# flanglet/kanzi-go

Measured on AMD Instinct MI355X. Metric: encode+decode MB/s (round trip of the whole stream, uncompressed 10^6 B per second), higher is better.
Workload: dtype u8

## Files before the change

kanzi-go_amd/csrc/ans1.hip:

```cpp
#include "bits.h"

#define KNZ_ANS1_CHUNK (4u << 20)
#define KNZ_ANS1_LR 11
#define KNZ_ANS1_SCALE 2048
#define KNZ_ANS1_LDS_MAX_CHUNKS 1280u
#define KNZ_ANS1_CTXHDR_BYTES 448
#define KNZ_ANS1_U0_CAP (256 * KNZ_ANS1_CTXHDR_BYTES + 64)
#define KNZ_ANS1_U1_OFF KNZ_ANS1_U0_CAP
#define KNZ_ANS1_PAY_OFF (KNZ_ANS1_U0_CAP + 64)
#define KNZ_ANS1_PAY_CAP (((KNZ_ANS1_CHUNK / 8) * 11) + 64)
#define KNZ_ANS1_SLOT (KNZ_ANS1_PAY_OFF + KNZ_ANS1_PAY_CAP + 64)
#define KNZ_ANS1_CUM_STRIDE 257
#define KNZ_ANS1_PAYRING 8192
#define KNZ_ANS1_RING 2048

struct Ans1Args {
    const uint64_t* blk_off;
    const uint32_t* blk_len;
    uint32_t chunks_per_block;
    uint32_t nslots;
    uint8_t* scratch;
    uint32_t* unit_bits;
    uint32_t* unit_src;
    uint32_t* freqs;
// ... 304 lines not shown
        flush(m0, m1, m2);
    }
    const uint32_t s1 = wave_shfl(st, 1), s2 = wave_shfl(st, 2), s3 = wave_shfl(st, 3);
    if (bad && lane == 0) a.blk_status[b] = KNZ_ERR_PROCESS_BLOCK;
    if (live && lane == 0) {
        const uint32_t end4 = n & ~3u;
        const uint32_t tail = n & 3;
        for (uint32_t i = 0; i < tail; i++) payEnd[i] = src[end4 + i];
        const uint32_t nbytes = 2 * flushed + tail;
        uint32_t w[8];
        for (int i = 0; i < 8; i++) w[i] = 0;
        KnzBitWriter bw;
        bw.init(w);
        knz_put_varint(bw, nbytes);
        bw.put(st, 32); bw.put(s1, 32); bw.put(s2, 32); bw.put(s3, 32);
        uint32_t* u1 = (uint32_t*)(slot + KNZ_ANS1_U1_OFF);
        for (int i = 0; i < 8; i++) u1[i] = knz_bswap32(w[i]);
        uint32_t* ubits = a.unit_bits + (size_t)slotId * KNZ_UNITS_PER_CHUNK;
        uint32_t* usrc = a.unit_src + (size_t)slotId * KNZ_UNITS_PER_CHUNK;
        ubits[1] = bw.pos;
        ubits[2] = 8 * nbytes;
        usrc[2] = (uint32_t)(KNZ_ANS1_PAY_OFF + KNZ_ANS1_PAY_CAP - 2 * flushed);
    }
}

#ifndef KNZ_HIP_EMU
#define KNZ_A1E_SDWA " dst_sel:DWORD dst_unused:UNUSED_PAD src0_sel:DWORD src1_sel:WORD_1\n\t"
#define KNZ_A1E_STEP(J, A, B) \
    "v_cmp_ge_u32_e32 vcc, %[" A "], %[y" J "]\n\t" \
    "v_cndmask_b32_sdwa %[t], %[" A "], %[" A "], vcc" KNZ_A1E_SDWA \
    "v_mul_hi_u32 %[q], %[t], %[x" J "]\n\t" \
    "v_lshrrev_b32_e32 %[q], %[w" J "], %[q]\n\t" \
    "v_mul_u32_u24_sdwa %[q], %[q], %[w" J "]" KNZ_A1E_SDWA \
    "v_add3_u32 %[" B "], %[t], %[z" J "], %[q]\n\t"
__device__ __forceinline__ void knz_a1e_run4(uint32_t& st, const uint4& e0, const uint4& e1, const uint4& e2, const uint4& e3, uint32_t* slot) {
    uint32_t q, t, s1, s2, s3, s4;
    asm volatile(KNZ_A1E_STEP("0", "s0", "s1") KNZ_A1E_STEP("1", "s1", "s2") KNZ_A1E_STEP("2", "s2", "s3") KNZ_A1E_STEP("3", "s3", "s4")
                 : [s1] "=&v"(s1), [s2] "=&v"(s2), [s3] "=&v"(s3), [s4] "=&v"(s4), [q] "=&v"(q), [t] "=&v"(t)
                 : [s0] "v"(st), [x0] "v"(e0.x), [y0] "v"(e0.y), [z0] "v"(e0.z), [w0] "v"(e0.w), [x1] "v"(e1.x), [y1] "v"(e1.y), [z1] "v"(e1.z), [w1] "v"(e1.w),
                   [x2] "v"(e2.x), [y2] "v"(e2.y), [z2] "v"(e2.z), [w2] "v"(e2.w), [x3] "v"(e3.x), [y3] "v"(e3.y), [z3] "v"(e3.z), [w3] "v"(e3.w)
                 : "vcc");
    uint4 sv; sv.x = st; sv.y = s1; sv.z = s2; sv.w = s3;
    *(uint4*)slot = sv;
    st = s4;
}
template <int R>
__device__ __forceinline__ void knz_a1e_run_group(uint32_t& st, const uint4* e, uint32_t* mine) {
    knz_a1e_run4(st, e[0], e[1], e[2], e[3], mine + R * 64);
    knz_a1e_run4(st, e[4], e[5], e[6], e[7], mine + R * 64 + 4);
    knz_a1e_run4(st, e[8], e[9], e[10], e[11], mine + R * 64 + 8);
    knz_a1e_run4(st, e[12], e[13], e[14], e[15], mine + R * 64 + 12);
}

__global__ __launch_bounds__(64) void knz_ans1_encode_asm_kernel(Ans1Args a, const uint4* ent) {
    __shared__ __attribute__((aligned(16))) uint32_t s_w[3 * KNZ_ANS1_GROUP * 4];
    const int lane = threadIdx.x;
    const uint32_t slotId = blockIdx.x;
    uint32_t b, n; const uint8_t* src; bool bad;
    const uint32_t steps = knz_ans1_steps(a, slotId, b, n, src, bad);
    const bool live = n != 0;
    uint8_t* slot = a.scratch + (size_t)slotId * KNZ_ANS1_SLOT;
    uint8_t* payEnd = slot + KNZ_ANS1_PAY_OFF + KNZ_ANS1_PAY_CAP;
    const uint4* __restrict__ base = ent + (size_t)slotId * KNZ_ANS1_ENT_STRIDE;
    const uint4* __restrict__ my = base + (size_t)(lane & 3);
    uint32_t* mine = s_w + 16 * (lane & 3);
    uint32_t st = 1u << 15;
    uint32_t flushed = 0;
    uint4 buf0[KNZ_ANS1_GROUP], buf1[KNZ_ANS1_GROUP], buf2[KNZ_ANS1_GROUP];
    uint32_t xm0 = 0xFFFFFFFFu, xm1 = 0xFFFFFFFFu, xm2;
    auto load_group = [&](uint32_t t0, uint4* e, uint32_t& xm) {
#pragma unroll
        for (int j = 0; j < KNZ_ANS1_GROUP; j++) e[j] = my[(size_t)(t0 + j) * 4];
        xm = base[(size_t)t0 * 4 + (uint32_t)lane].y;
    };
    auto flush = [&](uint32_t x0, uint32_t x1, uint32_t x2) {
        wave_sync_lds();
        const uint64_t below = ((uint64_t)1 << lane) - 1;
        const uint32_t fi = 16u * (uint32_t)(lane & 3) + (uint32_t)(lane >> 2);
        const uint32_t v0 = s_w[fi], v1 = s_w[64 + fi], v2 = s_w[128 + fi];
        const uint64_t m0 = wave_ballot(v0 >= x0), m1 = wave_ballot(v1 >= x1), m2 = wave_ballot(v2 >= x2);
        const uint32_t c0 = (uint32_t)__popcll(m0), c1 = (uint32_t)__popcll(m1), c2 = (uint32_t)__popcll(m2);
#pragma unroll
        for (int r = 0; r < 3; r++) {
            const uint64_t m = r == 0 ? m0 : (r == 1 ? m1 : m2);
            const uint32_t before = r == 0 ? 0u : (r == 1 ? c0 : c0 + c1);
            if ((m >> lane) & 1) {
                const uint32_t pos = flushed + before + (uint32_t)__popcll(m & below);
                const uint32_t wv = r == 0 ? v0 : (r == 1 ? v1 : v2);
                uint8_t* p = payEnd - 2 * ((size_t)pos + 1);
                p[0] = (uint8_t)(wv >> 8);
                p[1] = (uint8_t)wv;
            }
        }
        flushed += c0 + c1 + c2;
        wave_sync_lds();
    };
#pragma unroll
    for (int j = 0; j < KNZ_ANS1_GROUP; j++) { buf0[j].x = 0; buf0[j].y = 0xFFFFFFFFu; buf0[j].z = 0; buf0[j].w = 0; buf1[j] = buf0[j]; }
    for (uint32_t t0 = 0; t0 < steps + 2 * KNZ_ANS1_GROUP && steps; t0 += 3 * KNZ_ANS1_GROUP) {
        load_group(t0, buf2, xm2); knz_a1e_run_group<0>(st, buf0, mine);
        const uint32_t f0 = xm0;
        load_group(t0 + KNZ_ANS1_GROUP, buf0, xm0); knz_a1e_run_group<1>(st, buf1, mine);
        const uint32_t f1 = xm1;
        load_group(t0 + 2 * KNZ_ANS1_GROUP, buf1, xm1); knz_a1e_run_group<2>(st, buf2, mine);
        flush(f0, f1, xm2);
    }
    const uint32_t s1 = wave_shfl(st, 1), s2 = wave_shfl(st, 2), s3 = wave_shfl(st, 3);
    if (bad && lane == 0) a.blk_status[b] = KNZ_ERR_PROCESS_BLOCK;
    if (live && lane == 0) {
        const uint32_t end4 = n & ~3u;
        const uint32_t tail = n & 3;
        for (uint32_t i = 0; i < tail; i++) payEnd[i] = src[end4 + i];
        const uint32_t nbytes = 2 * flushed + tail;
        uint32_t w[8];
        for (int i = 0; i < 8; i++) w[i] = 0;
        KnzBitWriter bw;
        bw.init(w);
        knz_put_varint(bw, nbytes);
        bw.put(st, 32); bw.put(s1, 32); bw.put(s2, 32); bw.put(s3, 32);
        uint32_t* u1 = (uint32_t*)(slot + KNZ_ANS1_U1_OFF);
        for (int i = 0; i < 8; i++) u1[i] = knz_bswap32(w[i]);
        uint32_t* ubits = a.unit_bits + (size_t)slotId * KNZ_UNITS_PER_CHUNK;
        uint32_t* usrc = a.unit_src + (size_t)slotId * KNZ_UNITS_PER_CHUNK;
        ubits[1] = bw.pos;
        ubits[2] = 8 * nbytes;
        usrc[2] = (uint32_t)(KNZ_ANS1_PAY_OFF + KNZ_ANS1_PAY_CAP - 2 * flushed);
    }
}
#endif

struct Ans1DecArgs {
    const uint8_t* stream; uint64_t nbytes;
    const uint32_t* blk_pre_len;
    const uint8_t* blk_mode;
    const uint64_t* chunk_bit;
    const uint64_t* blk_out_off;
    uint32_t chunks_per_block;
    uint32_t nslots;
    uint32_t* dtab;
    uint32_t* info;
    uint64_t* paybit;
    int32_t* blk_status;
    uint32_t plain_loop;
    uint64_t* progress;
};

template <typename R>
__device__ static bool knz_ans1_parse_ctx(R& r, uint16_t* f, uint32_t llr, uint32_t scale, int& countOut) {
    uint8_t alpha[256];
    int count = 0;
    if (r.read(1) == 0) {
        if (r.read(1) == 1) count = 0;
        else { count = 256; if (f) for (int i = 0; i < 256; i++) alpha[i] = (uint8_t)i; }
    } else {
        const uint32_t lastMask = r.read(5);
        if (f) {
            for (uint32_t mm = 0; mm <= lastMask; mm++) {
                const uint32_t mask = r.read(8);
                for (int j = 0; j < 8; j++) if ((mask >> j) & 1) alpha[count++] = (uint8_t)(8 * mm + j);
            }
        } else {
            for (uint32_t bitsLeft = 8 * (lastMask + 1); bitsLeft > 0;) {
                const uint32_t take = bitsLeft > 32 ? 32 : bitsLeft;
                count += __popc(r.read(take));
                bitsLeft -= take;
            }
        }
    }
    countOut = count;
    if (count == 0) return true;
    const int chk = count < 64 ? 6 : 8;
    uint32_t sum = 0;
    for (int i = 1; i < count; i += chk) {
        const uint32_t logMax = r.read(llr);
        if ((1u << logMax) > scale) return false;
        const int endj = min(i + chk, count);
        if (!f) { r.skip_bits((uint32_t)(endj - i) * logMax); continue; }
        for (int j = i; j < endj; j++) {
            uint32_t fr = 1;
            if (logMax > 0) { fr = 1 + r.read(logMax); if (fr >= scale) return false; }
            f[alpha[j]] = (uint16_t)fr;
            sum += fr;
// ... 598 lines not shown
```

kanzi-go_amd/csrc/huffman_dec.hip:

```cpp
#include "bits.h"

struct KnzStreamReader {
    const uint32_t* words;
    uint64_t nwords;
    uint64_t next;
    uint64_t win;
    uint32_t navail;
    uint32_t pre;
    __device__ __forceinline__ uint32_t ld_raw(uint64_t i) const { return i < nwords ? words[i] : 0u; }
    __device__ __forceinline__ uint32_t ld(uint64_t i) const { return knz_bswap32(ld_raw(i)); }
    __device__ __forceinline__ void init(const uint8_t* base, uint64_t nbytes, uint64_t bitpos) {
        words = (const uint32_t*)base;
        nwords = (nbytes + 3) >> 2;
        uint64_t q = bitpos >> 5;
        uint32_t off = (uint32_t)(bitpos & 31);
        win = ((uint64_t)ld(q) << 32) | ld(q + 1);
        win <<= off;
        navail = 64 - off;
        next = q + 2;
        pre = ld_raw(next);
    }
    __device__ __forceinline__ void refill() {
        if (navail <= 32) { win |= (uint64_t)knz_bswap32(pre) << (32 - navail); navail += 32; next++; pre = ld_raw(next); }
    }
// ... 15 lines not shown
    uint64_t win;
    uint32_t navail;
    __device__ __forceinline__ void stage(uint64_t b) {
        const uint64_t l = (uint64_t)lane_id();
        base = b;
        w0 = (b + l < nwords) ? words[b + l] : 0u;
        w1 = (b + 64 + l < nwords) ? words[b + 64 + l] : 0u;
    }
    __device__ __forceinline__ uint32_t ld(uint64_t i) {
        if (i < base || i >= base + 128) stage(i);
        const uint32_t k = (uint32_t)(i - base);
        const uint32_t v = k < 64 ? wave_readlane(w0, k) : wave_readlane(w1, k - 64);
        return knz_bswap32(v);
    }
    __device__ __forceinline__ void init(const uint8_t* b, uint64_t nbytes, uint64_t bitpos) {
        words = (const uint32_t*)b;
        nwords = (nbytes + 3) >> 2;
        stage(bitpos >> 5);
        seek(bitpos);
    }
    __device__ __forceinline__ void seek(uint64_t bitpos) {
        const uint64_t q = bitpos >> 5;
        const uint32_t off = (uint32_t)(bitpos & 31);
        win = ((uint64_t)ld(q) << 32) | ld(q + 1);
        win <<= off;
        navail = 64 - off;
        next = q + 2;
    }
    __device__ __forceinline__ void refill() {
        if (navail <= 32) { win |= (uint64_t)ld(next++) << (32 - navail); navail += 32; }
    }
    __device__ __forceinline__ uint32_t peek(uint32_t n) { refill(); return (uint32_t)(win >> (64 - n)); }
    __device__ __forceinline__ void skip(uint32_t n) { refill(); win <<= n; navail -= n; }
    __device__ __forceinline__ void skip_bits(uint32_t n) { if (n <= 32) skip(n); else seek(tell() + n); }
    __device__ __forceinline__ uint32_t read(uint32_t n) { uint32_t v = peek(n); win <<= n; navail -= n; return v; }
    __device__ __forceinline__ uint64_t tell() const { return (next << 5) - navail; }
};

template <typename R>
__device__ __forceinline__ uint32_t knz_read_varint(R& r) {
    uint32_t res = 0, shift = 0;
    for (int i = 0; i < 4; i++) {
        uint32_t v = r.read(8);
        res |= (v & 0x7F) << shift;
        if (v < 128) return res;
        shift += 7;
    }
    uint32_t v = r.read(8);
    return res | ((v & 0x0F) << 28);
}

template <typename R>
__device__ static bool knz_ans1_parse_header(R& r, uint16_t* freq16, uint32_t& lrOut, int& totalAlpha, uint64_t* ctxpos, bool store);

struct WalkStreamArgs {
    const uint8_t* stream; uint64_t nbytes;
    uint64_t first_bit;
    uint64_t seg_bits;
    uint32_t max_blocks;
    uint64_t* blk_bit;
    uint64_t* blk_bits;
    uint32_t* result;
};

__global__ void knz_dec_walk_stream_kernel(WalkStreamArgs a) {
    if (threadIdx.x != 0 || blockIdx.x != 0) return;
    KnzStreamReader r;
    r.init(a.stream, a.nbytes, a.first_bit);
    const uint64_t limit = a.nbytes << 3;
    uint32_t n = 0, err = 0;
    for (;;) {
        if (a.seg_bits && r.tell() >= a.first_bit + a.seg_bits) break;
        if (r.tell() + 8 > limit) { err = KNZ_ERR_PROCESS_BLOCK; break; }
        uint32_t lr = r.read(5) + 3;
        uint64_t read = 0;
        if (lr > 32) { read = (uint64_t)r.read(lr - 32) << 32; read |= r.read(32); }
        else read = r.read(lr);
        if (read == 0) break;
        if (read > ((uint64_t)1 << 34)) { err = KNZ_ERR_BLOCK_SIZE; break; }
        uint64_t pos = r.tell();
        if (pos + read > limit) { err = KNZ_ERR_PROCESS_BLOCK; break; }
        if (n >= a.max_blocks) { err = KNZ_ERR_BLOCK_SIZE; break; }
        a.blk_bit[n] = pos;
        a.blk_bits[n] = read;
        n++;
        r.seek(pos + read);
    }
    a.result[0] = n;
    a.result[1] = err;
}

struct WalkRangeArgs {
    const uint8_t* stream; uint64_t nbytes;
    uint64_t first_bit;
    uint64_t first_id, from, to;
    uint32_t max_blocks;
    uint32_t cap;
    uint32_t frames;
    uint32_t stride;
    uint32_t hinted;
    uint64_t* blk_bit; uint64_t* blk_bits;
    uint64_t* result;
};

__global__ void knz_dec_walk_range_kernel(WalkRangeArgs a) {
    if (threadIdx.x != 0 || blockIdx.x != 0) return;
    KnzStreamReader r;
    r.init(a.stream, a.nbytes, a.first_bit);
    const uint64_t limit = a.nbytes << 3;
    uint64_t id = a.first_id, n = 0, end = 0;
    uint32_t seen = 0, err = 0;
    while (id < a.to) {
        const uint64_t at = r.tell();
        if (at + 8 > limit) { err = KNZ_ERR_PROCESS_BLOCK; break; }
        const uint32_t lr = r.read(5) + 3;
        uint64_t read = 0;
        if (lr > 32) { read = (uint64_t)r.read(lr - 32) << 32; read |= r.read(32); }
        else read = r.read(lr);
        const uint64_t pos = r.tell();
        if (read == 0) { end = pos; if (a.hinted && seen == 0) err = KNZ_ERR_PROCESS_BLOCK; break; }
        if (read > ((uint64_t)1 << 34)) { err = KNZ_ERR_BLOCK_SIZE; break; }
        if (pos + read > limit) { err = KNZ_ERR_PROCESS_BLOCK; break; }
        if (seen >= a.max_blocks) { err = KNZ_ERR_BLOCK_SIZE; break; }
        seen++;
        if (id >= a.from) {
            if (n < a.cap) { a.blk_bit[n * a.stride] = a.frames ? at : pos; a.blk_bits[n * a.stride] = read; }
            n++;
        }
        id++;
        r.seek(pos + read);
    }
    a.result[0] = n;
    a.result[1] = err;
    a.result[2] = end;
}

struct WalkBlocksArgs {
    const uint8_t* stream; uint64_t nbytes;
    const uint64_t* blk_bit; const uint64_t* blk_bits;
    uint32_t nblocks;
    uint32_t block_size;
    uint32_t checksum_bits;
    uint32_t entropy;
    uint32_t chunks_per_block;
    uint32_t payload_only;
    uint32_t given_len;
    uint32_t* blk_pre_len;
    uint8_t* blk_mode;
    uint8_t* blk_skip;
    uint64_t* blk_cksum;
    uint64_t* chunk_bit;
    int32_t* blk_status;
    uint64_t* blk_end_bit;
    uint32_t check_out;
    uint64_t* out_off;
    uint64_t out_base, out_stride, out_cap;
    uint32_t stream_block_size;
    uint64_t* ans1_ctx_bit;
};

template <typename R>
__device__ __forceinline__ void knz_skip_expg(R& r) {
    uint32_t w = r.peek(17);
    if (w & 0x10000) { r.skip(1); return; }
    if (w == 0) { r.skip(17); return; }
    uint32_t z = (uint32_t)__builtin_clz(w << 15);
    uint32_t lg = z & 7;
    r.skip(z + 1);
    r.skip(lg + 1);
}

#define KNZ_EXPG_WIN 12
__device__ __forceinline__ uint32_t knz_expg_lut_entry(uint32_t w) {
    uint32_t pos = 0, codes = 0;
    while (pos < KNZ_EXPG_WIN) {
        if ((w >> (KNZ_EXPG_WIN - 1 - pos)) & 1) { codes++; pos++; continue; }
        uint32_t z = 0;
        while (pos + z < KNZ_EXPG_WIN && !((w >> (KNZ_EXPG_WIN - 1 - pos - z)) & 1)) z++;
        if (pos + z >= KNZ_EXPG_WIN) break;
        const uint32_t total = z + 1 + (z & 7) + 1;
        if (pos + total > KNZ_EXPG_WIN) break;
        codes++; pos += total;
    }
    return (codes << 4) | pos;
}

struct HufDecArgs {
    const uint8_t* stream; uint64_t nbytes;
    const uint32_t* blk_pre_len;
    const uint8_t* blk_mode;
    const uint64_t* chunk_bit;
    const uint64_t* blk_out_off;
    uint32_t chunks_per_block;
    uint32_t entropy;
    uint8_t* out;
    int32_t* blk_status;
};

__global__ __launch_bounds__(64) void knz_huf_decode_kernel(HufDecArgs a, const uint8_t* only) {
    __shared__ uint16_t s_table[1 << KNZ_HUF_MAXLEN];
    __shared__ uint8_t s_len[256];
    __shared__ uint8_t s_alpha[256];
    __shared__ uint16_t s_C[256];
    __shared__ uint8_t s_symAt[256];
    __shared__ uint32_t s_fragbits[4];
    __shared__ uint64_t s_fragpos[4];
    __shared__ int s_count, s_err;
    __shared__ uint64_t s_tailpos;

    const int lane = threadIdx.x;
    if (only && !only[blockIdx.x]) return;
// ... 153 lines not shown
```

kanzi-go_amd/csrc/huffman_par.hip:

```cpp
#include "bits.h"

#ifdef KNZ_PROFILE_PHASES
__device__ unsigned long long g_knz_prof[32];
#define KNZ_PROF_T(var) const unsigned long long var = __builtin_readcyclecounter()
#define KNZ_PROF_ADD(i, a, b) do { if (threadIdx.x == 0) atomicAdd(&g_knz_prof[i], (b) - (a)); } while (0)
#define KNZ_PROF_INC(i, v) do { if (threadIdx.x == 0) atomicAdd(&g_knz_prof[i], (unsigned long long)(v)); } while (0)
#else
#define KNZ_PROF_INC(i, v)
#define KNZ_PROF_T(var)
#define KNZ_PROF_ADD(i, a, b)
#endif

#define KNZ_HUF_SYNC_BITS 192
#define KNZ_HUF_LANE_CAP 84
#define KNZ_HW_WORDS 136

struct KnzHufHdr {
    uint32_t count;
    uint32_t fb[4];
    uint32_t end;
    uint32_t status;
};

struct KnzLinWin {
// ... 563 lines not shown
        const uint32_t chunkSize = (a.entropy == KNZ_E_ANS1 || a.entropy == KNZ_E_FPAQ) ? (4u << 20) : (uint32_t)KNZ_HUF_CHUNK;
        const uint32_t nchunks = (preLen + chunkSize - 1) / chunkSize;
        if (nchunks > cpb) status = KNZ_ERR_BLOCK_SIZE;
        const uint32_t* swords = (const uint32_t*)a.stream;
        const uint64_t snwords = (a.nbytes + 3) >> 2;
        uint64_t pos = r.tell();
        bool stale = false;
        uint32_t filled = 0;
        for (uint32_t k = 0; k < nchunks && status == 0; k++) {
            const uint32_t sz = min(chunkSize, preLen - k * chunkSize);
            if (writer) knz_publish64(&a.chunk_bit[(size_t)b * cpb + k], pos);
            published = k + 1;
            if (entropy == KNZ_E_HUFFMAN && sz >= 32 && ringLive) {
                KNZ_PROF_T(w0);
                const uint64_t w0i = pos >> 5;
                const uint32_t rel = (uint32_t)(w0i - ringOrigin);
                if (writer) vsync[1] = rel;
                const uint32_t need = (uint32_t)min((uint64_t)rel + KNZ_HW_WORDS, ((snwords - ringOrigin + 255) & ~(uint64_t)255));
                if (filled < need) {
                    uint32_t spins = 0;
                    while ((filled = vsync[0]) < need) { wave_spin_pause(); if (++spins > (1u << 24)) break; }
                    if (filled < need) ringLive = false;
                    else wg_fence_acquire();
                }
              if (ringLive) {
                KNZ_PROF_T(w1);
                KNZ_PROF_T(w2);
                const KnzHufHdr hdr = knz_huf_parse_header_wave<false>(KnzRingWin{s_ring, rel, KNZ_WALK_RING - 1}, (uint32_t)(pos & 31), nullptr, nullptr, (int)threadIdx.x);
                KNZ_PROF_T(w3);
                KNZ_PROF_T(w4);
                KNZ_PROF_ADD(8, w0, w1); KNZ_PROF_ADD(9, w1, w2); KNZ_PROF_ADD(10, w2, w3); KNZ_PROF_ADD(11, w3, w4);
                if (hdr.status == 2) { status = KNZ_ERR_PROCESS_BLOCK; break; }
                if (hdr.status == 0) {
                    uint64_t np = (w0i << 5) + hdr.end;
                    if (hdr.count > 1) {
                        if ((int32_t)(hdr.fb[0] | hdr.fb[1] | hdr.fb[2] | hdr.fb[3]) < 0) status = KNZ_ERR_PROCESS_BLOCK;
                        np += (uint64_t)hdr.fb[0] + hdr.fb[1] + hdr.fb[2] + hdr.fb[3] + 8ull * (sz & 3);
                    }
                    pos = np;
                    stale = true;
                    if (pos > limit) status = KNZ_ERR_PROCESS_BLOCK;
                    continue;
                }
              }
            }
            if (stale) { r.seek(pos); stale = false; }
            if (entropy == KNZ_E_NONE || (entropy == KNZ_E_HUFFMAN && sz < 32) || ((entropy == KNZ_E_ANS0 || entropy == KNZ_E_ANS1) && preLen <= 32)) {
                r.seek(r.tell() + 8ull * sz);
            } else if (entropy == KNZ_E_FPAQ) {
                const uint32_t szb = knz_read_varint(r);
                if ((int32_t)szb < 0 || (uint64_t)szb >= 2ull * preLen) status = KNZ_ERR_PROCESS_BLOCK;
                r.seek(r.tell() + 56 + 8ull * szb);
            } else if (entropy == KNZ_E_ANS1) {
                uint32_t lr; int total;
                if (!knz_ans1_parse_header(r, nullptr, lr, total, a.ans1_ctx_bit ? a.ans1_ctx_bit + ((size_t)b * cpb + k) * 257 : nullptr, writer) || total == 0) { status = KNZ_ERR_PROCESS_BLOCK; break; }
                const uint32_t szb = knz_read_varint(r);
                if (szb >= (1u << 27)) status = KNZ_ERR_PROCESS_BLOCK;
                r.seek(r.tell() + 128 + 8ull * szb);
            } else if (entropy == KNZ_E_ANS0) {
                const uint32_t lr = 8 + r.read(3);
                uint32_t llr = 3;
                while ((1u << llr) <= lr) llr++;
                uint32_t count;
                if (r.read(1) == 0) count = r.read(1) == 1 ? 0 : 256;
                else {
                    uint32_t lastMask = r.read(5);
                    count = 0;
                    for (uint32_t m = 0; m <= lastMask; m++) count += (uint32_t)__popc(r.read(8));
                }
                if (count == 0) { status = KNZ_ERR_PROCESS_BLOCK; break; }
                const uint32_t chk = count < 64 ? 6 : 8;
                for (uint32_t i = 1; i < count; i += chk) {
                    const uint32_t logMax = r.read(llr);
                    const uint32_t endj = min(i + chk, count);
                    if (logMax > 16) { status = KNZ_ERR_PROCESS_BLOCK; break; }
                    r.seek(r.tell() + (uint64_t)(endj - i) * logMax);
                }
                if (count > 1 && status == 0) {
                    const uint32_t szb = knz_read_varint(r);
                    if (szb >= (1u << 27)) status = KNZ_ERR_PROCESS_BLOCK;
                    r.seek(r.tell() + 128 + 8ull * szb);
                }
            } else {
                uint32_t count;
                if (r.read(1) == 0) {
                    if (r.read(1) == 1) { status = KNZ_ERR_PROCESS_BLOCK; break; }
                    count = 256;
                } else {
                    uint32_t lastMask = r.read(5);
                    count = 0;
                    for (uint32_t bitsLeft = 8 * (lastMask + 1); bitsLeft > 0;) {
                        const uint32_t take = bitsLeft > 32 ? 32 : bitsLeft;
                        count += (uint32_t)__popc(r.read(take));
                        bitsLeft -= take;
                    }
                    if (count == 0) { status = KNZ_ERR_PROCESS_BLOCK; break; }
                }
                for (uint32_t i = 0; i < count;) {
                    const uint32_t e = s_lut[r.peek(KNZ_EXPG_WIN)];
                    const uint32_t nc = e >> 4;
                    if (nc == 0 || i + nc > count) { knz_skip_expg(r); i++; }
                    else { r.skip(e & 15); i += nc; }
                }
                if (count > 1) {
                    uint64_t fb = 0;
                    for (int j = 0; j < 4; j++) {
                        uint32_t v = knz_read_varint(r);
                        if ((int32_t)v < 0) status = KNZ_ERR_PROCESS_BLOCK;
// ... 59 lines not shown
```

kanzi-go_amd/csrc/knz_batch.inc:

```

struct EncodeBatch {
    const uint8_t* d_src; uint64_t n;
    uint8_t* d_dst; uint64_t dst_cap;
    int framed = 0, with_header = 0, with_end = 0; int64_t header_input_size = 0;
    uint64_t out_stride = 0;
    int payload_only = 0;
    int keep_probes = 0;
    uint64_t total_bits = 0;
    struct Many { const ManyStream* streams = nullptr; uint32_t n_streams = 0, blocks = 0, max_len = 0; uint32_t* blk_stream = nullptr; } many;
    static EncodeBatch stream(const uint8_t* src, uint64_t n, uint8_t* dst, uint64_t cap, int64_t header_input_size) {
        EncodeBatch eb = segment(src, n, dst, cap); eb.with_header = eb.with_end = 1; eb.header_input_size = header_input_size; return eb;
    }
    static EncodeBatch segment(const uint8_t* src, uint64_t n, uint8_t* dst, uint64_t cap) { EncodeBatch eb(src, n, dst, cap); eb.framed = 1; return eb; }
    static EncodeBatch block_streams(const uint8_t* src, uint64_t n, uint8_t* dst, uint64_t stride, uint64_t count) {
        EncodeBatch eb(src, n, dst, stride * count + 64); eb.out_stride = stride; return eb;
    }
    static EncodeBatch payload(const uint8_t* src, uint64_t n, uint8_t* dst, uint64_t cap) { EncodeBatch eb = block_streams(src, n, dst, cap, 1); eb.payload_only = 1; return eb; }
private:
    EncodeBatch(const uint8_t* src, uint64_t nn, uint8_t* dst, uint64_t cap) : d_src(src), n(nn), d_dst(dst), dst_cap(cap) {}
};

struct DecodeBatch {
    const uint8_t* d_stream; uint64_t nbytes;
    int framed;
// ... 26 lines not shown
    HufEncArgs hufArgs;
};

template <class A> static void enc_io(A& a, Handle* h, uint32_t cpb) {
    a.blk_off = h->blk_off.as<uint64_t>(); a.blk_len = h->blk_len.as<uint32_t>(); a.chunks_per_block = cpb;
    a.scratch = h->scratch.as<uint8_t>(); a.unit_bits = h->unit_bits.as<uint32_t>(); a.unit_src = h->unit_src.as<uint32_t>();
    a.blk_status = h->blk_status.as<int32_t>();
}
template <class A> static void enc_group(A& a, uint32_t b0, size_t s0, uint32_t slotStride) {
    a.blk_off += b0; a.blk_len += b0; a.blk_status += b0;
    a.scratch += s0 * slotStride; a.unit_bits += s0 * KNZ_UNITS_PER_CHUNK; a.unit_src += s0 * KNZ_UNITS_PER_CHUNK;
}

static int huf_encode_stage(Handle* h, EncStage& s, hipStream_t st) {
    const uint32_t nblocks = s.nblocks, cpb = s.cpb;
    HufEncArgs a;
    enc_io(a, h, cpb); a.data = nullptr;
    if (h->cfg.entropy == KNZ_E_HUFFMAN) {
        const uint32_t nc = nblocks * cpb, groups = (nc + 63) / 64;
        if (h->huf_stfreq.reserve((size_t)groups * 256 * 64 * 2) || h->huf_stsym.reserve((size_t)groups * 256 * 64) ||
            h->huf_stlen.reserve((size_t)groups * 256 * 64) || h->huf_stcnt.reserve((size_t)groups * 64 * 2) || h->huf_stmax.reserve((size_t)groups * 64))
            return knz_set_error(h, KNZ_ERR_CREATE_COMPRESSOR, "device workspace allocation failed");
        a.st_freq = h->huf_stfreq.as<uint16_t>(); a.st_sym = h->huf_stsym.as<uint8_t>(); a.st_len = h->huf_stlen.as<uint8_t>();
        a.st_count = h->huf_stcnt.as<uint16_t>(); a.st_maxlen = h->huf_stmax.as<uint8_t>(); a.nchunks = nc;
        s.hufDirect = !s.skipOpt && knz_test_switch("KNZ_HUF_SCRATCH") == nullptr;
        a.st_fhist = nullptr; a.dst_words = nullptr; a.chunk_rel = nullptr; a.blk_dst_bit = nullptr; a.total_bits = nullptr;
        if (s.hufDirect) {
            if (h->huf_fhist.reserve((size_t)nc * 4 * 256 * 2 + 64)) return knz_set_error(h, KNZ_ERR_CREATE_COMPRESSOR, "device workspace allocation failed");
            a.st_fhist = h->huf_fhist.as<uint16_t>();
        }
        KNZ_LAUNCH_PROBED(knz_huf_hist_kernel, dim3(nc), dim3(256), 0, st, a);
        KNZ_LAUNCH_PROBED(knz_huf_lengths_kernel, dim3(groups), dim3(64), 0, st, a);
        if (s.hufDirect) { KNZ_LAUNCH_PROBED(knz_huf_encode_kernel<true>, dim3(nc), dim3(256), 0, st, a); s.hufArgs = a; }
        else KNZ_LAUNCH_PROBED(knz_huf_encode_kernel<false>, dim3(nc), dim3(256), 0, st, a);
    }
    else hipLaunchKernelGGL(knz_raw_units_kernel, dim3(nblocks * cpb), dim3(256), 0, st, a);
    return KNZ_OK;
}

static int fpaq_encode_stage(Handle* h, EncStage& s, hipStream_t st) {
    FpaqArgs a;
    enc_io(a, h, s.cpb); a.blk_src_len = h->blk_src_len.as<uint32_t>();
    KNZ_LAUNCH_PROBED(knz_fpaq_encode_kernel, dim3(s.nblocks), dim3(64), 0, st, a);
    return KNZ_OK;
}

static int ans1_encode_stage(Handle* h, EncStage& s, hipStream_t st) {
    const uint32_t nblocks = s.nblocks, cpb = s.cpb;
    const size_t perSlot = (size_t)65536 * 12 + (size_t)256 * KNZ_ANS1_CTXHDR_BYTES + 1024 + KNZ_ANS1_ENT_STRIDE * 16;
    const uint32_t slotsPerGroup = (uint32_t)std::max<size_t>(cpb, std::min<size_t>((size_t)nblocks * cpb, ((size_t)64 << 30) / perSlot));
    uint32_t GB = std::max<uint32_t>(1, slotsPerGroup / cpb);
    if (const char* e = knz_test_switch("KNZ_ANS1_GROUP_BLOCKS")) GB = std::max(1, atoi(e));
    const bool ans1EncPlain = knz_test_switch("KNZ_ANS1_ENC_PLAIN") != nullptr;
    uint32_t gs = GB * cpb;
    for (;;) {
        gs = GB * cpb;
        if (!(h->a1_freqs.reserve((size_t)gs * 65536 * 4) || h->a1_tab.reserve((size_t)gs * 65536 * 8) ||
              h->a1_ctxhdr.reserve((size_t)gs * 256 * KNZ_ANS1_CTXHDR_BYTES + 64) || h->a1_ctxbits.reserve((size_t)gs * 256 * 4) ||
              h->a1_ent.reserve((size_t)gs * KNZ_ANS1_ENT_STRIDE * 16)))
            break;
        if (GB == 1) return knz_set_error(h, KNZ_ERR_CREATE_COMPRESSOR, "device workspace allocation failed");
        h->a1_freqs.release(); h->a1_tab.release(); h->a1_ctxhdr.release(); h->a1_ctxbits.release(); h->a1_ent.release();
        GB = (GB + 1) / 2;
    }
    for (uint32_t b0 = 0; b0 < nblocks; b0 += GB) {
        const uint32_t gb = std::min<uint32_t>(GB, nblocks - b0), ns = gb * cpb;
        const size_t s0 = (size_t)b0 * cpb;
        Ans1Args a;
        enc_io(a, h, cpb); enc_group(a, b0, s0, s.slotStride); a.nslots = ns;
        a.freqs = h->a1_freqs.as<uint32_t>(); a.tab = h->a1_tab.as<uint2>(); a.ctx_hdr = h->a1_ctxhdr.as<uint8_t>();
        a.ctx_bits = h->a1_ctxbits.as<uint32_t>();
        hipMemsetAsync(h->a1_freqs.p, 0, (size_t)ns * 65536 * 4, st);
        KNZ_LAUNCH_PROBED(knz_ans1_hist_kernel, dim3(ns * KNZ_ANS1_HIST_WGS * KNZ_ANS1_HIST_SLICES), dim3(256), 0, st, a);
        hipLaunchKernelGGL(knz_ans1_stats_kernel, dim3(ns * 256), dim3(64), 0, st, a);
        hipLaunchKernelGGL(knz_ans1_merge_kernel, dim3(ns), dim3(256), 0, st, a);
        KNZ_LAUNCH_PROBED(knz_ans1_expand_kernel, dim3(ns, 128), dim3(256), 0, st, a, h->a1_ent.as<uint4>());
#ifndef KNZ_HIP_EMU
        if (!ans1EncPlain) KNZ_LAUNCH_PROBED(knz_ans1_encode_asm_kernel, dim3(ns), dim3(64), 0, st, a, (const uint4*)h->a1_ent.as<uint4>());
        else
#endif
        KNZ_LAUNCH_PROBED(knz_ans1_encode_kernel, dim3(ns), dim3(64), 0, st, a, (const uint4*)h->a1_ent.as<uint4>());
    }
    return KNZ_OK;
}

static int ans0_encode_stage(Handle* h, EncStage& s, hipStream_t st) {
    Ans0Args a;
    enc_io(a, h, s.cpb); a.data = nullptr;
    a.tab = h->ans_tab.as<uint2>(); a.chunk_info = (uint32_t*)(h->ans_tab.as<uint8_t>() + s.nslots * 2048);
    const uint32_t ns = s.nblocks * s.cpb;
    hipLaunchKernelGGL(knz_ans0_stats_kernel, dim3(ns), dim3(256), 0, st, a);
    KNZ_LAUNCH_PROBED(knz_ans0_encode_kernel, dim3((ns + KNZ_ANS0_CHUNKS_PER_WG - 1) / KNZ_ANS0_CHUNKS_PER_WG), dim3(128), 0, st, a, ns);
    return KNZ_OK;
}

#define KNZ_PIPE_DEVICE_BLOCKS 1024
#include <atomic>
static std::atomic<int> g_pipe_blocks[64];
struct PipeScope {
    Handle* h;
    int blocks = 0;
    bool launched = false;
    explicit PipeScope(Handle* hh) : h(hh) {}
    bool take(int n) {
        const int dev = h->device & 63;
        if (g_pipe_blocks[dev].fetch_add(n) + n > KNZ_PIPE_DEVICE_BLOCKS) { g_pipe_blocks[dev].fetch_sub(n); return false; }
        blocks = n;
        return true;
    }
    ~PipeScope() {
        if (launched) { hipStreamSynchronize(h->stream2); hipStreamSynchronize(h->stream3); }
        if (blocks) g_pipe_blocks[h->device & 63].fetch_sub(blocks);
    }
};

struct RankPipe {
    PipeScope scope;
    bool on = false, groups = false;
    RankPipeArgs args{};
    uint8_t* take[2] = {nullptr, nullptr};
    explicit RankPipe(Handle* h) : scope(h) {}
};

struct DecStage {
    DecodeBatch& db;
    uint32_t nblocks, cpb; size_t nslots;
    WalkBlocksArgs wb;
    bool fusedWalk, direct, xf;
    XfBatch xb; uint64_t xstride = 0;
    RankPipe pipe;
    DecStage(Handle* h, DecodeBatch& b) : db(b), pipe(h) {}
};

template <class A> static void dec_io(A& a, const DecodeBatch& db, Handle* h, uint32_t cpb) {
// ... 369 lines not shown
        WalkRangeArgs wr;
        wr.stream = db.d_stream; wr.nbytes = db.nbytes; wr.first_bit = db.first_bit; wr.first_id = db.rg_first_id; wr.from = db.rg_from; wr.to = db.rg_to;
        wr.max_blocks = walkBound; wr.cap = maxBlocks; wr.frames = 0; wr.stride = 1; wr.hinted = db.rg_hinted ? 1 : 0;
        wr.blk_bit = blkBit.as<uint64_t>(); wr.blk_bits = blkBits.as<uint64_t>(); wr.result = h->total_bits.as<uint64_t>();
        hipLaunchKernelGGL(knz_dec_walk_range_kernel, dim3(1), dim3(1), 0, st, wr);
        uint64_t* res = (uint64_t*)h->pinned;
        HIP_OK(hipMemcpyAsync(res, h->total_bits.p, 24, hipMemcpyDeviceToHost, st));
        HIP_OK(hipStreamSynchronize(st));
        if (res[1]) return knz_set_error(h, (int)res[1], "invalid block framing in stream");
        nblocks = (uint32_t)res[0];
    } else if (db.framed) {
        WalkStreamArgs ws;
        ws.stream = db.d_stream; ws.nbytes = db.nbytes; ws.first_bit = db.first_bit; ws.seg_bits = db.seg_bits; ws.max_blocks = maxBlocks;
        ws.blk_bit = blkBit.as<uint64_t>(); ws.blk_bits = blkBits.as<uint64_t>(); ws.result = h->total_bits.as<uint32_t>();
        hipLaunchKernelGGL(knz_dec_walk_stream_kernel, dim3(1), dim3(1), 0, st, ws);
        uint32_t* res = (uint32_t*)h->pinned;
        HIP_OK(hipMemcpyAsync(res, h->total_bits.p, 8, hipMemcpyDeviceToHost, st));
        HIP_OK(hipStreamSynchronize(st));
        if (res[1]) return knz_set_error(h, (int)res[1], "invalid block framing in stream");
        nblocks = res[0];
    }
    db.nblocks = nblocks;
    db.total_out = 0;
    db.pre_len.assign(nblocks, 0); db.end_bit.assign(nblocks, 0); db.status.assign(nblocks, 0);
    return KNZ_OK;
}

static int dec_header_pass(Handle* h, DecStage& d, const EntropyCodec& ec, hipStream_t st) {
    const DecodeBatch& db = d.db;
    const uint32_t nblocks = d.nblocks = db.nblocks;
    WalkBlocksArgs& wb = d.wb;
    const uint32_t maxPre = db.payload_only ? db.given_len : knz_max_encoded_len(db.transform, db.block_size);
    const uint32_t cpb = d.cpb = std::max<uint32_t>(1, (maxPre + ec.chunk - 1) / ec.chunk);
    const size_t nslots = d.nslots = (size_t)nblocks * cpb;
    if (h->blk_len.reserve(4 * (size_t)nblocks) || h->blk_skip.reserve(2 * (size_t)nblocks + 16) || h->blk_cksum.reserve(8 * (size_t)nblocks) ||
        h->chunk_rel.reserve(8 * nslots) || h->blk_status.reserve(4 * (size_t)nblocks) || h->blk_off.reserve(8 * (size_t)nblocks) ||
        h->dec_tables.reserve(8 * (size_t)nblocks))
        return knz_set_error(h, KNZ_ERR_CREATE_DECOMPRESSOR, "device workspace allocation failed");
    hipEventRecord(h->ev[0], st);
    wb.stream = db.d_stream; wb.nbytes = db.nbytes; wb.blk_bit = h->blk_dst_bit.as<uint64_t>(); wb.blk_bits = h->blk_written.as<uint64_t>();
    wb.nblocks = nblocks;
    wb.block_size = db.block_size + std::max<uint32_t>(512, db.block_size >> 4);
    wb.checksum_bits = db.checksum_bits; wb.entropy = db.entropy; wb.chunks_per_block = cpb;
    wb.payload_only = db.payload_only; wb.given_len = db.given_len;
    wb.blk_pre_len = h->blk_len.as<uint32_t>(); wb.blk_mode = h->blk_skip.as<uint8_t>(); wb.blk_skip = h->blk_skip.as<uint8_t>() + nblocks;
    wb.blk_cksum = h->blk_cksum.as<uint64_t>(); wb.chunk_bit = h->chunk_rel.as<uint64_t>(); wb.blk_status = h->blk_status.as<int32_t>();
    wb.blk_end_bit = h->dec_tables.as<uint64_t>();
    const bool fusedWalk = d.fusedWalk = (db.entropy == KNZ_E_HUFFMAN || db.entropy == KNZ_E_ANS0) && knz_test_switch("KNZ_HUF_SPLIT_WALK") == nullptr;
    d.xf = db.transform != 0 && !db.payload_only;
    const bool direct = d.direct = fusedWalk && !d.xf;
    wb.check_out = direct ? 1 : 0; wb.out_off = h->blk_off.as<uint64_t>(); wb.out_base = (uint64_t)db.d_out; wb.out_stride = db.out_stride;
    wb.out_cap = db.out_cap; wb.stream_block_size = db.block_size;
    wb.ans1_ctx_bit = nullptr;
    if (db.entropy == KNZ_E_ANS1) {
        if (h->a1_ctxpos.reserve((size_t)nslots * 257 * 8 + 64)) return knz_set_error(h, KNZ_ERR_CREATE_DECOMPRESSOR, "device workspace allocation failed");
        wb.ans1_ctx_bit = h->a1_ctxpos.as<uint64_t>();
    }
    if (fusedWalk) hipLaunchKernelGGL(knz_dec_block_headers_kernel, dim3(nblocks), dim3(64), 0, st, wb);
    else hipLaunchKernelGGL(knz_dec_walk_blocks_kernel, dim3(nblocks), dim3(128), 0, st, wb);
    hipEventRecord(h->ev[1], st);
    return KNZ_OK;
}

static int dec_block_fits(Handle* h, const DecodeBatch& db, uint32_t b) {
    if (db.pre_len[b] > db.block_size || (db.pre_len[b] > db.out_stride && b + 1 < db.nblocks))
        return knz_set_error(h, KNZ_ERR_PROCESS_BLOCK, "block decodes to more than the stream block size");
    if ((uint64_t)b * db.out_stride + db.pre_len[b] > db.out_cap) return knz_set_error(h, KNZ_ERR_WRITE_FILE, "destination buffer too small");
    return KNZ_OK;
}

static int dec_place_outputs(Handle* h, DecStage& d, hipStream_t st) {
    DecodeBatch& db = d.db;
    XfBatch& xb = d.xb;
    const uint32_t nblocks = d.nblocks;
    const bool xf = d.xf;
    uint64_t& xstride = d.xstride;
    if (xf) {
        const uint64_t padded = (uint64_t)db.block_size + std::max<uint32_t>(512, db.block_size >> 4);
        xstride = (std::max<uint64_t>(knz_max_encoded_len(db.transform, db.block_size), padded) + 64 + 15) & ~(uint64_t)15;
        if (xf_alloc(h, xb, nblocks, xstride)) return knz_set_error(h, KNZ_ERR_CREATE_DECOMPRESSOR, "device workspace allocation failed");
        xb.ctx_entropy = db.entropy; xb.ctx_block_size = db.block_size;
    }
    std::vector<uint64_t> off(nblocks);
    for (uint32_t b = 0; b < nblocks; b++) off[b] = xf ? (uint64_t)h->xf_r1.p + (uint64_t)b * xstride : (uint64_t)db.d_out + (uint64_t)b * db.out_stride;
    HIP_OK(hipMemcpyAsync(h->blk_off.p, off.data(), 8 * (size_t)nblocks, hipMemcpyHostToDevice, st));
    HIP_OK(hipMemcpyAsync(db.pre_len.data(), h->blk_len.p, 4 * (size_t)nblocks, hipMemcpyDeviceToHost, st));
    HIP_OK(hipMemcpyAsync(db.status.data(), h->blk_status.p, 4 * (size_t)nblocks, hipMemcpyDeviceToHost, st));
    HIP_OK(hipStreamSynchronize(st));
    int first = KNZ_OK;
    for (uint32_t b = 0; b < nblocks; b++) {
        int rc = KNZ_OK;
        if (db.status[b]) rc = knz_set_error(h, db.status[b], "invalid block in stream");
        else if (xf) { if (db.pre_len[b] > xstride) rc = knz_set_error(h, KNZ_ERR_BLOCK_SIZE, "block larger than the decoder buffers"); }
        else rc = dec_block_fits(h, db, b);
        if (rc && db.block_failed(b, rc, first)) return rc;
    }
    return first;
}

static int dec_inverse_transforms(Handle* h, DecStage& d, hipStream_t st) {
    DecodeBatch& db = d.db;
    XfBatch& xb = d.xb;
    const RankPipe& pipe = d.pipe;
    const uint32_t nblocks = d.nblocks;
    if (!pipe.on) {
        std::vector<uint8_t> ones(nblocks, 1);
// ... 89 lines not shown
```

Measured before the change: 387.1.

## Split ANS1 encode into producer/consumer waves and walk decode headers wave-wide

The ANS1 encoder now runs two waves per workgroup. One wave runs the serial state recurrence and writes pre-renormalisation states into an 8-slot LDS ring. The other wave polls LDS flags, ballots which states flush, and writes the 16-bit payload words, so the serial chain no longer waits on output compaction. The old single-wave kernel stays behind a switch. Separately, the ANS1 context-header walk on the decode side uses a wave-cooperative bit window (readlane, and popcount via scan) instead of a serial bit reader. The price is spin-wait handshakes with timeouts, more threads per workgroup, and added code complexity.

```diff
diff --git a/kanzi-go_amd/csrc/ans1.hip b/kanzi-go_amd/csrc/ans1.hip
--- a/kanzi-go_amd/csrc/ans1.hip
+++ b/kanzi-go_amd/csrc/ans1.hip
@@ -380,7 +380,7 @@
     knz_a1e_run4(st, e[12], e[13], e[14], e[15], mine + R * 64 + 12);
 }
 
-__global__ __launch_bounds__(64) void knz_ans1_encode_asm_kernel(Ans1Args a, const uint4* ent) {
+__global__ __launch_bounds__(64) void knz_ans1_encode_asm1_kernel(Ans1Args a, const uint4* ent) {
     __shared__ __attribute__((aligned(16))) uint32_t s_w[3 * KNZ_ANS1_GROUP * 4];
     const int lane = threadIdx.x;
     const uint32_t slotId = blockIdx.x;
@@ -456,6 +456,160 @@
     }
 }
 #endif
+
+#define KNZ_A1E_RING 8
+#define KNZ_A1E_TURN (3 * KNZ_ANS1_GROUP)
+#define KNZ_A1E_SPINS (1u << 24)
+#ifndef KNZ_HIP_EMU
+__device__ __forceinline__ uint32_t knz_lds_poll(const uint32_t* p) { return __hip_atomic_load(p, __ATOMIC_RELAXED, __HIP_MEMORY_SCOPE_WORKGROUP); }
+__device__ __forceinline__ void knz_lds_post(uint32_t* p, uint32_t v) { __hip_atomic_store(p, v, __ATOMIC_RELAXED, __HIP_MEMORY_SCOPE_WORKGROUP); }
+#else
+inline uint32_t knz_lds_poll(const uint32_t* p) { return *(const volatile uint32_t*)p; }
+inline void knz_lds_post(uint32_t* p, uint32_t v) { *(volatile uint32_t*)p = v; }
+#endif
+struct __attribute__((aligned(16))) KnzA1eShared {
+    uint32_t ring[KNZ_A1E_RING][KNZ_A1E_TURN * 4];
+    uint32_t fin[4];
+    uint32_t sync[4];
+};
+
+#ifdef KNZ_HIP_EMU
+template <int R>
+__device__ __forceinline__ void knz_a1e_run_group(uint32_t& st, const uint4* e, uint32_t* mine) {
+#pragma unroll
+    for (int j = 0; j < KNZ_ANS1_GROUP; j++) {
+        mine[R * 64 + j] = st;
+        st = st >= e[j].y ? (st >> 16) : st;
+        const uint32_t qq = (uint32_t)(((uint64_t)st * e[j].x) >> 32) >> (e[j].w & 31u);
+        st = st + e[j].z + knz_mul24(qq, e[j].w >> 16);
+    }
+}
+#endif
+
+__global__ __launch_bounds__(128) void knz_ans1_encode_asm_kernel(Ans1Args a, const uint4* ent) {
+    __shared__ KnzA1eShared sh;
+    const int lane = threadIdx.x & 63;
+    const uint32_t slotId = blockIdx.x;
+    uint32_t b, n; const uint8_t* src; bool bad;
+    const uint32_t steps = knz_ans1_steps(a, slotId, b, n, src, bad);
+    const bool live = n != 0;
+    const uint32_t nturns = steps ? (steps + 2 * KNZ_ANS1_GROUP + KNZ_A1E_TURN - 1) / KNZ_A1E_TURN : 0u;
+    const uint4* __restrict__ base = ent + (size_t)slotId * KNZ_ANS1_ENT_STRIDE;
+    if (threadIdx.x < 4) sh.sync[threadIdx.x] = 0;
+    __syncthreads();
+    if (threadIdx.x < 64) {
+        const uint4* __restrict__ my = base + (size_t)(lane & 3);
+        uint32_t st = 1u << 15;
+        uint4 buf0[KNZ_ANS1_GROUP], buf1[KNZ_ANS1_GROUP], buf2[KNZ_ANS1_GROUP];
+        auto load_group = [&](const uint4* g, uint4* e) {
+#pragma unroll
+            for (int j = 0; j < KNZ_ANS1_GROUP; j++) e[j] = g[j * 4];
+        };
+#pragma unroll
+        for (int j = 0; j < KNZ_ANS1_GROUP; j++) { buf0[j].x = 0; buf0[j].y = 0xFFFFFFFFu; buf0[j].z = 0; buf0[j].w = 0; buf1[j] = buf0[j]; }
+        uint32_t placed = 0;
+        uint32_t slot = 0;
+        bool gaveUp = false;
+        for (uint32_t turn = 0; turn < nturns; turn++) {
+            if (turn >= placed + KNZ_A1E_RING) {
+                uint32_t spins = 0;
+                while (turn >= (placed = knz_lds_poll(&sh.sync[1])) + KNZ_A1E_RING) {
+                    if (knz_lds_poll(&sh.sync[3]) != 0 || ++spins > KNZ_A1E_SPINS) { gaveUp = true; break; }
+                    wave_spin_pause();
+                }
+                if (gaveUp) break;
+            }
+            const uint32_t seen = knz_lds_poll(&sh.sync[1]);
+            uint32_t* mine = sh.ring[slot] + 16 * (lane & 3);
+            load_group(my, buf2); knz_a1e_run_group<0>(st, buf0, mine);
+            load_group(my + 4 * KNZ_ANS1_GROUP, buf0); knz_a1e_run_group<1>(st, buf1, mine);
+            load_group(my + 8 * KNZ_ANS1_GROUP, buf1); knz_a1e_run_group<2>(st, buf2, mine);
+            my += 4 * KNZ_A1E_TURN;
+            wave_sync_lds();
+            knz_lds_post(&sh.sync[0], turn + 1);
+            placed = seen;
+            slot = slot + 1 == KNZ_A1E_RING ? 0 : slot + 1;
+        }
+        if (lane < 4) sh.fin[lane] = st;
+        wave_sync_lds();
+        if (gaveUp) knz_lds_post(&sh.sync[3], 1u);
+        knz_lds_post(&sh.sync[2], 1u);
+        return;
+    }
+    uint8_t* slotMem = a.scratch + (size_t)slotId * KNZ_ANS1_SLOT;
+    uint8_t* payEnd = slotMem + KNZ_ANS1_PAY_OFF + KNZ_ANS1_PAY_CAP;
+    uint32_t flushed = 0;
+    bool gaveUp = false;
+    const uint64_t below = ((uint64_t)1 << lane) - 1;
+    const uint32_t fi = 16u * (uint32_t)(lane & 3) + (uint32_t)(lane >> 2);
+    auto xmax = [&](uint32_t turn, uint32_t g) -> uint32_t {
+        const uint32_t t = turn * KNZ_A1E_TURN + g * KNZ_ANS1_GROUP;
+        return (turn < nturns && t >= 2 * KNZ_ANS1_GROUP) ? base[(size_t)(t - 2 * KNZ_ANS1_GROUP) * 4 + (uint32_t)lane].y : 0xFFFFFFFFu;
+    };
+    uint32_t xa[3], xb[3], xc[3];
+#pragma unroll
+    for (uint32_t g = 0; g < 3; g++) { xa[g] = xmax(0, g); xb[g] = xmax(1, g); xc[g] = xmax(2, g); }
+    uint32_t slot = 0;
+    for (uint32_t turn = 0; turn < nturns; turn++) {
+        uint32_t spins = 0;
+        while (knz_lds_poll(&sh.sync[0]) <= turn) {
+            if (knz_lds_poll(&sh.sync[3]) != 0 || ++spins > KNZ_A1E_SPINS) { gaveUp = true; break; }
+            wave_spin_pause();
+        }
+        if (gaveUp) break;
+        wave_sync_lds();
+        const uint32_t* w = sh.ring[slot];
+        const uint32_t v0 = knz_lds_poll(w + fi), v1 = knz_lds_poll(w + 64 + fi), v2 = knz_lds_poll(w + 128 + fi);
+        const uint64_t m0 = wave_ballot(v0 >= xa[0]), m1 = wave_ballot(v1 >= xa[1]), m2 = wave_ballot(v2 >= xa[2]);
+        wave_sync_lds();
+        knz_lds_post(&sh.sync[1], turn + 1);
+        const uint32_t c0 = (uint32_t)__popcll(m0), c1 = (uint32_t)__popcll(m1), c2 = (uint32_t)__popcll(m2);
+#pragma unroll
+        for (int r = 0; r < 3; r++) {
+            const uint64_t m = r == 0 ? m0 : (r == 1 ? m1 : m2);
+            const uint32_t before = r == 0 ? 0u : (r == 1 ? c0 : c0 + c1);
+            if ((m >> lane) & 1) {
+                const uint32_t pos = flushed + before + (uint32_t)__popcll(m & below);
+                const uint32_t wv = r == 0 ? v0 : (r == 1 ? v1 : v2);
+                uint8_t* p = payEnd - 2 * ((size_t)pos + 1);
+                p[0] = (uint8_t)(wv >> 8);
+                p[1] = (uint8_t)wv;
+            }
+        }
+        flushed += c0 + c1 + c2;
+#pragma unroll
+        for (uint32_t g = 0; g < 3; g++) { xa[g] = xb[g]; xb[g] = xc[g]; xc[g] = xmax(turn + 3, g); }
+        slot = slot + 1 == KNZ_A1E_RING ? 0 : slot + 1;
+    }
+    if (gaveUp) knz_lds_post(&sh.sync[3], 1u);
+    for (uint32_t spins = 0; !gaveUp && knz_lds_poll(&sh.sync[2]) == 0;) {
+        if (++spins > KNZ_A1E_SPINS) { gaveUp = true; knz_lds_post(&sh.sync[3], 1u); break; }
+        wave_spin_pause();
+    }
+    wave_sync_lds();
+    if (knz_lds_poll(&sh.sync[3]) != 0) gaveUp = true;
+    if ((bad || (gaveUp && live)) && lane == 0) a.blk_status[b] = KNZ_ERR_PROCESS_BLOCK;
+    if (live && !gaveUp && lane == 0) {
+        const uint32_t st = knz_lds_poll(&sh.fin[0]), s1 = knz_lds_poll(&sh.fin[1]), s2 = knz_lds_poll(&sh.fin[2]), s3 = knz_lds_poll(&sh.fin[3]);
+        const uint32_t end4 = n & ~3u;
+        const uint32_t tail = n & 3;
+        for (uint32_t i = 0; i < tail; i++) payEnd[i] = src[end4 + i];
+        const uint32_t nbytes = 2 * flushed + tail;
+        uint32_t w[8];
+        for (int i = 0; i < 8; i++) w[i] = 0;
+        KnzBitWriter bw;
+        bw.init(w);
+        knz_put_varint(bw, nbytes);
+        bw.put(st, 32); bw.put(s1, 32); bw.put(s2, 32); bw.put(s3, 32);
+        uint32_t* u1 = (uint32_t*)(slotMem + KNZ_ANS1_U1_OFF);
+        for (int i = 0; i < 8; i++) u1[i] = knz_bswap32(w[i]);
+        uint32_t* ubits = a.unit_bits + (size_t)slotId * KNZ_UNITS_PER_CHUNK;
+        uint32_t* usrc = a.unit_src + (size_t)slotId * KNZ_UNITS_PER_CHUNK;
+        ubits[1] = bw.pos;
+        ubits[2] = 8 * nbytes;
+        usrc[2] = (uint32_t)(KNZ_ANS1_PAY_OFF + KNZ_ANS1_PAY_CAP - 2 * flushed);
+    }
+}
 
 struct Ans1DecArgs {
     const uint8_t* stream; uint64_t nbytes;
diff --git a/kanzi-go_amd/csrc/huffman_dec.hip b/kanzi-go_amd/csrc/huffman_dec.hip
--- a/kanzi-go_amd/csrc/huffman_dec.hip
+++ b/kanzi-go_amd/csrc/huffman_dec.hip
@@ -91,6 +91,102 @@
 
 template <typename R>
 __device__ static bool knz_ans1_parse_header(R& r, uint16_t* freq16, uint32_t& lrOut, int& totalAlpha, uint64_t* ctxpos, bool store);
+
+#define KNZ_A1W_STEP 48u
+struct KnzAns1Walk {
+    const uint32_t* words;
+    uint64_t nwords;
+    uint64_t base;
+    uint32_t rp;
+    uint32_t wa, wb;
+    uint32_t na, nb;
+    int lane;
+    __device__ __forceinline__ void load(uint64_t wbase, uint32_t& x, uint32_t& y) const {
+        const uint64_t i = wbase + (uint64_t)lane;
+        if (wbase + 65 <= nwords) { x = words[i]; y = words[i + 1]; }
+        else { x = i < nwords ? words[i] : 0u; y = i + 1 < nwords ? words[i + 1] : 0u; }
+    }
+    __device__ __forceinline__ void init(const uint8_t* s, uint64_t nbytes, uint64_t bitpos) {
+        words = (const uint32_t*)s;
+        nwords = (nbytes + 3) >> 2;
+        lane = lane_id();
+        base = ((uint64_t)wave_uniform((uint32_t)(bitpos >> 37)) << 32) | wave_uniform((uint32_t)(bitpos >> 5));
+        rp = wave_uniform((uint32_t)bitpos & 31u);
+        uint32_t x, y;
+        load(base, x, y);
+        wa = knz_bswap32(x); wb = knz_bswap32(y);
+        load(base + KNZ_A1W_STEP, na, nb);
+    }
+    __device__ __forceinline__ void shift() {
+        wa = knz_bswap32(na); wb = knz_bswap32(nb);
+        base += KNZ_A1W_STEP;
+        rp -= 32u * KNZ_A1W_STEP;
+        load(base + KNZ_A1W_STEP, na, nb);
+    }
+    __device__ __forceinline__ uint64_t fetch() const {
+        const uint32_t k = rp >> 5;
+        return (((uint64_t)wave_readlane(wa, k) << 32) | wave_readlane(wb, k)) << (rp & 31u);
+    }
+    __device__ __forceinline__ uint64_t tell() const { return (base << 5) + rp; }
+    __device__ __forceinline__ uint32_t popcount_bits(uint32_t nbits) const {
+        const int s = (int)rp - 32 * lane, e = s + (int)nbits;
+        const uint32_t lo = (uint32_t)min(max(s, 0), 32), hi = (uint32_t)min(max(e, 0), 32);
+        const uint32_t m = (uint32_t)(0xFFFFFFFF00000000ull >> hi) & (uint32_t)(0xFFFFFFFFull >> lo);
+        return wave_readlane(wave_scan_incl((uint32_t)__popc(wa & m)), 63);
+    }
+};
+
+__device__ static bool knz_ans1_walk_header(const uint8_t* stream, uint64_t nbytes, uint64_t pos, uint64_t* ctxpos, int& totalAlpha, uint64_t& endpos) {
+    KnzAns1Walk w;
+    w.init(stream, nbytes, pos);
+    const uint64_t origin = w.base << 5;
+    uint32_t moved = 0;
+    const uint32_t lr = 8 + (uint32_t)(w.fetch() >> 61);
+    w.rp += 3;
+    totalAlpha = 0;
+    endpos = pos;
+    if (lr > 16) return false;
+    uint32_t llr = 3;
+    while ((1u << llr) <= lr) llr++;
+    uint32_t mine = 0;
+    uint32_t total = 0;
+    bool ok = true;
+    int k = 0;
+    for (; k < 256 && ok; k++) {
+        if (__builtin_expect(w.rp >= 32u * 54u, 0)) do { w.shift(); moved += 32u * KNZ_A1W_STEP; } while (w.rp >= 32u * 54u);
+        if (w.lane == (k & 63)) mine = moved + w.rp;
+        const uint64_t h = w.fetch();
+        uint32_t count;
+        if ((h >> 63) == 0) { count = ((h >> 62) & 1) ? 0u : 256u; w.rp += 2; }
+        else {
+            const uint32_t nbits = 8u * (((uint32_t)(h >> 58) & 31u) + 1u);
+            w.rp += 6;
+            count = w.popcount_bits(nbits);
+            w.rp += nbits;
+        }
+        total += count;
+        if (count > 1) {
+            const uint32_t chk = count < 64 ? 6u : 8u;
+            uint32_t widest = 0;
+            uint32_t left = count - 1;
+            do {
+                if (__builtin_expect(w.rp >= 32u * 64u, 0)) do { w.shift(); moved += 32u * KNZ_A1W_STEP; } while (w.rp >= 32u * 64u);
+                const uint32_t logMax = (uint32_t)(w.fetch() >> (64 - llr));
+                const uint32_t n = min(chk, left);
+                widest = max(widest, logMax);
+                w.rp += llr + n * logMax;
+                left -= n;
+            } while (left != 0);
+            ok = widest <= lr;
+        }
+        if (ctxpos && ((k & 63) == 63 || !ok)) { if (w.lane <= (k & 63)) ctxpos[(k & ~63) + w.lane] = origin + mine; }
+    }
+    totalAlpha = (int)total;
+    if (!ok) return false;
+    endpos = origin + moved + w.rp;
+    if (ctxpos && w.lane == 0) ctxpos[256] = endpos;
+    return true;
+}
 
 struct WalkStreamArgs {
     const uint8_t* stream; uint64_t nbytes;
@@ -196,6 +292,7 @@
     uint64_t out_base, out_stride, out_cap;
     uint32_t stream_block_size;
     uint64_t* ans1_ctx_bit;
+    uint32_t ans1_walk_plain;
 };
 
 template <typename R>
diff --git a/kanzi-go_amd/csrc/huffman_par.hip b/kanzi-go_amd/csrc/huffman_par.hip
--- a/kanzi-go_amd/csrc/huffman_par.hip
+++ b/kanzi-go_amd/csrc/huffman_par.hip
@@ -639,8 +639,16 @@
                 if ((int32_t)szb < 0 || (uint64_t)szb >= 2ull * preLen) status = KNZ_ERR_PROCESS_BLOCK;
                 r.seek(r.tell() + 56 + 8ull * szb);
             } else if (entropy == KNZ_E_ANS1) {
-                uint32_t lr; int total;
-                if (!knz_ans1_parse_header(r, nullptr, lr, total, a.ans1_ctx_bit ? a.ans1_ctx_bit + ((size_t)b * cpb + k) * 257 : nullptr, writer) || total == 0) { status = KNZ_ERR_PROCESS_BLOCK; break; }
+                int total;
+                uint64_t* ctxpos = a.ans1_ctx_bit ? a.ans1_ctx_bit + ((size_t)b * cpb + k) * 257 : nullptr;
+                if (a.ans1_walk_plain) {
+                    uint32_t lr;
+                    if (!knz_ans1_parse_header(r, nullptr, lr, total, ctxpos, writer) || total == 0) { status = KNZ_ERR_PROCESS_BLOCK; break; }
+                } else {
+                    uint64_t hdrEnd;
+                    if (!knz_ans1_walk_header(a.stream, a.nbytes, r.tell(), ctxpos, total, hdrEnd) || total == 0) { status = KNZ_ERR_PROCESS_BLOCK; break; }
+                    r.seek(hdrEnd);
+                }
                 const uint32_t szb = knz_read_varint(r);
                 if (szb >= (1u << 27)) status = KNZ_ERR_PROCESS_BLOCK;
                 r.seek(r.tell() + 128 + 8ull * szb);
diff --git a/kanzi-go_amd/csrc/knz_batch.inc b/kanzi-go_amd/csrc/knz_batch.inc
--- a/kanzi-go_amd/csrc/knz_batch.inc
+++ b/kanzi-go_amd/csrc/knz_batch.inc
@@ -102,6 +102,7 @@
     uint32_t GB = std::max<uint32_t>(1, slotsPerGroup / cpb);
     if (const char* e = knz_test_switch("KNZ_ANS1_GROUP_BLOCKS")) GB = std::max(1, atoi(e));
     const bool ans1EncPlain = knz_test_switch("KNZ_ANS1_ENC_PLAIN") != nullptr;
+    const bool ans1EncOneWave = knz_test_switch("KNZ_ANS1_ENC_ONE_WAVE") != nullptr;
     uint32_t gs = GB * cpb;
     for (;;) {
         gs = GB * cpb;
@@ -125,11 +126,11 @@
         hipLaunchKernelGGL(knz_ans1_stats_kernel, dim3(ns * 256), dim3(64), 0, st, a);
         hipLaunchKernelGGL(knz_ans1_merge_kernel, dim3(ns), dim3(256), 0, st, a);
         KNZ_LAUNCH_PROBED(knz_ans1_expand_kernel, dim3(ns, 128), dim3(256), 0, st, a, h->a1_ent.as<uint4>());
+        if (!ans1EncPlain && !ans1EncOneWave) KNZ_LAUNCH_PROBED(knz_ans1_encode_asm_kernel, dim3(ns), dim3(128), 0, st, a, (const uint4*)h->a1_ent.as<uint4>());
 #ifndef KNZ_HIP_EMU
-        if (!ans1EncPlain) KNZ_LAUNCH_PROBED(knz_ans1_encode_asm_kernel, dim3(ns), dim3(64), 0, st, a, (const uint4*)h->a1_ent.as<uint4>());
-        else
+        else if (!ans1EncPlain) KNZ_LAUNCH_PROBED(knz_ans1_encode_asm1_kernel, dim3(ns), dim3(64), 0, st, a, (const uint4*)h->a1_ent.as<uint4>());
 #endif
-        KNZ_LAUNCH_PROBED(knz_ans1_encode_kernel, dim3(ns), dim3(64), 0, st, a, (const uint4*)h->a1_ent.as<uint4>());
+        else KNZ_LAUNCH_PROBED(knz_ans1_encode_kernel, dim3(ns), dim3(64), 0, st, a, (const uint4*)h->a1_ent.as<uint4>());
     }
     return KNZ_OK;
 }
@@ -605,6 +606,7 @@
     wb.check_out = direct ? 1 : 0; wb.out_off = h->blk_off.as<uint64_t>(); wb.out_base = (uint64_t)db.d_out; wb.out_stride = db.out_stride;
     wb.out_cap = db.out_cap; wb.stream_block_size = db.block_size;
     wb.ans1_ctx_bit = nullptr;
+    wb.ans1_walk_plain = knz_test_switch("KNZ_ANS1_WALK_PLAIN") != nullptr ? 1u : 0u;
     if (db.entropy == KNZ_E_ANS1) {
         if (h->a1_ctxpos.reserve((size_t)nslots * 257 * 8 + 64)) return knz_set_error(h, KNZ_ERR_CREATE_DECOMPRESSOR, "device workspace allocation failed");
         wb.ans1_ctx_bit = h->a1_ctxpos.as<uint64_t>();
```

New measurement: 391.3 (median of 6 runs). +1.1%, better.
